# lmb-freiburg/demon

Measured on NVIDIA H100. Metric: image_pairs_per_sec_256x192, higher is better.
Workload: dtype tf32x3

## Files before the change

### demon_b200/_lib.py

```python
import ctypes
import os

_HERE = os.path.dirname(os.path.abspath(__file__))
_DEFAULT = os.path.join(_HERE, "lib", "libdemon_b200.so")

c_void_p, c_int, c_int64, c_float, c_double, c_char_p = (
    ctypes.c_void_p, ctypes.c_int, ctypes.c_int64, ctypes.c_float, ctypes.c_double, ctypes.c_char_p)

_P = c_void_p
PROTOTYPES = {
    "demon_warp2d_f32": [_P, _P, _P, c_int, c_int, c_int, c_int, c_int, c_int, c_float, _P],
    "demon_warp2d_f64": [_P, _P, _P, c_int, c_int, c_int, c_int, c_int, c_int, c_double, _P],
    "demon_depth_to_flow_f32": [_P, _P, _P, _P, _P, c_int, c_int, c_int, c_int, c_int, c_int, _P],
    "demon_depth_to_flow_f64": [_P, _P, _P, _P, _P, c_int, c_int, c_int, c_int, c_int, c_int, _P],
    "demon_flow_to_depth_f32": [_P, _P, _P, _P, _P, c_int, c_int, c_int, c_int, c_int, c_int, _P],
    "demon_flow_to_depth_f64": [_P, _P, _P, _P, _P, c_int, c_int, c_int, c_int, c_int, c_int, _P],
    "demon_leaky_relu_f32": [_P, _P, c_int64, c_float, _P],
    "demon_leaky_relu_f64": [_P, _P, c_int64, c_double, _P],
    "demon_median3x3_downsample_f32": [_P, _P, c_int64, c_int, c_int, _P],
    "demon_median3x3_downsample_f64": [_P, _P, c_int64, c_int, c_int, _P],
    "demon_scale_invariant_gradient_f32": [_P, _P, c_int64, c_int, c_int, _P, _P, c_int, c_float, _P],
    "demon_scale_invariant_gradient_f64": [_P, _P, c_int64, c_int, c_int, _P, _P, c_int, c_double, _P],
    "demon_scale_invariant_gradient_grad_f32": [_P, _P, _P, c_int64, c_int, c_int, _P, _P, c_int, c_float, _P],
    "demon_scale_invariant_gradient_grad_f64": [_P, _P, _P, c_int64, c_int, c_int, _P, _P, c_int, c_double, _P],
# ... 82 lines not shown
    "demon_net_batch": [_P],
    "demon_net_workspace_bytes": [_P],
    "demon_net_pipeline_launches": [_P, c_int],
    "demon_net_snapshot_launches": [_P, c_int],
    "demon_net_layer_uses_tensor_cores": [_P, c_char_p],
    "demon_net_profile_begin": [_P],
    "demon_net_profile_end": [_P],
    "demon_net_num_layers": [_P],
    "demon_net_layer_name": [_P, c_int],
    "demon_net_layer_profile": [_P, c_int, _P, _P, _P, _P],
    "demon_debug_tc_timeouts": [],
    "demon_check_errors": [],
    "demon_debug_describe_layers": [_P, _P, c_int],
    "demon_debug_trace_layers": [_P, _P, _P],
    "demon_debug_describe_conv": [c_int] * 13 + [_P, c_int],
    "demon_debug_last_conv_ms": [],
    "demon_debug_tc_timing": [c_int, _P, c_int],
    "demon_conv_slice_nhwc": [_P, c_int, _P] + [c_int] * 11 + [_P, _P, c_int, c_int, _P],
    "demon_conv_slice_nhwc_same": [_P, c_int, _P] + [c_int] * 10 + [_P, _P, c_int, c_int, _P],
    "demon_conv2d_nhwc": [_P, _P] + [c_int] * 9 + [_P, _P, c_int, c_int, _P],
    "demon_deconv4x4s2_nhwc": [_P, _P] + [c_int] * 5 + [_P, _P, c_int, c_int, _P],
    "demon_last_error": [],
    "demon_version": [],
    "demon_launch_count": [],
}
_RESTYPES = {
    "demon_net_destroy": None,
    "demon_net_variable_name": c_char_p,
    "demon_net_layer_name": c_char_p,
    "demon_net_workspace_bytes": c_int64,
# ... 47 lines not shown
```

### demon_b200/csrc/conv_tc.cuh

```cuda
#pragma once
#include "conv.cuh"

namespace demon {

struct HaloPlan;

struct TcLayer {
  HaloPlan* plan = nullptr;
  size_t splitk_bytes = 0;
  bool per_tap = false;
};

constexpr int kTcNoPlan = 1;

int tc_prepare(TcLayer& t, const ConvProblem* probs, const float* const* w_hosts, int nclass, int precision);
int conv_tc_launch(const TcLayer& t, const ConvProblem* probs, cudaStream_t stream);
int tc_describe(const ConvProblem* probs, int nclass, int precision, char* buf, int buflen);
void tc_layer_free(TcLayer& t);
int tc_read_error_flag(bool clear);
void tc_halo_enable_timing(bool on);
int tc_halo_read_timing(long long* host, int nblocks);

}
```

### demon_b200/csrc/conv_tc_halo.cu

```cuda
#include <cuda.h>

#include <algorithm>
#include <cstring>
#include <memory>
#include <mutex>
#include <vector>

#include "conv_tc.cuh"
#include "conv_tc_ptx.cuh"
#include "wgmma_tf32.cuh"

namespace demon {

namespace {

constexpr int kRing = 4;
constexpr int kThreads = 384;
constexpr int kConsumerWarps = 8;
constexpr int kMaxAStages = 4;
constexpr int kTileH = 16, kTileW = 8;
constexpr int kMaxPlanes = 4;
constexpr int kPlanSms = 132;
constexpr int kSmemBudget = 224 * 1024;
constexpr int kMaxDynSmem = 226 * 1024;
// ... 48 lines not shown
__device__ __forceinline__ void wait_t(uint32_t bar, uint32_t parity, int* err, long long& acc) {
  if (mbar_try(bar, parity)) return;
  const long long t0 = clock64();
  for (;;) {
    if (mbar_try(bar, parity)) break;
    if (clock64() - t0 > kTimeoutCycles || *reinterpret_cast<volatile int*>(err) != 0) {
      atomicExch(err, 1);
      break;
    }
  }
  acc += clock64() - t0;
}

__device__ __forceinline__ int fast_div(int x, int d, uint32_t mul) { return mul ? (int)__umulhi((uint32_t)x, mul) : x; }

template <bool PER_TAP>
__device__ __forceinline__ void halo_decode_tile(const HaloParams& p, int tile, int& nt, int& n, int& y0, int& x0) {
  int m = fast_div(tile, p.n_tiles, p.mul_n_tiles);
  nt = tile - m * p.n_tiles;
  const int m1 = fast_div(m, p.tiles_x, p.mul_tiles_x);
  const int xb = m - m1 * p.tiles_x;
  n = fast_div(m1, p.tiles_y, p.mul_tiles_y);
  const int yb = m1 - n * p.tiles_y;
  if (PER_TAP) { n *= p.tb; y0 = yb * p.th; x0 = xb * p.tw; }
  else { y0 = yb * kTileH; x0 = xb * kTileW; }
}

template <int N, int MODE>
__device__ __forceinline__ void issue_block(float* acc, const uint32_t* hi, const uint32_t* lo, uint32_t wb) {
  const uint64_t w_hi = wgmma_desc_sw128(wb);
  const uint64_t w_lo = wgmma_desc_sw128(wb + N * 128u);
#pragma unroll
  for (int j = 0; j < 4; ++j) {
    if (MODE == 2) {
      Wgmma<N>::mma(acc, hi[4 * j], hi[4 * j + 1], hi[4 * j + 2], hi[4 * j + 3], w_lo + (uint64_t)(2 * j));
      Wgmma<N>::mma(acc, lo[4 * j], lo[4 * j + 1], lo[4 * j + 2], lo[4 * j + 3], w_hi + (uint64_t)(2 * j));
    }
    Wgmma<N>::mma(acc, hi[4 * j], hi[4 * j + 1], hi[4 * j + 2], hi[4 * j + 3], w_hi + (uint64_t)(2 * j));
  }
}

template <bool PER_TAP, bool CIN8, int MODE, int N, int NCLS>
__global__ void __launch_bounds__(kThreads, 1) conv_tc_halo_kernel(const __grid_constant__ HaloMaps maps, const HaloParams p) {
  extern __shared__ __align__(1024) unsigned char smem_raw[];
  unsigned char* smem = reinterpret_cast<unsigned char*>((reinterpret_cast<uintptr_t>(smem_raw) + 1023) & ~(uintptr_t)1023);
  __shared__ __align__(8) uint64_t bars[2 * kMaxAStages + 2 * kRing + 1];

  const int warp = threadIdx.x >> 5;
  const int lane = threadIdx.x & 31;
  const uint32_t afull0 = smem_u32(&bars[0]), aempty0 = smem_u32(&bars[kMaxAStages]);
  const uint32_t wfull0 = smem_u32(&bars[2 * kMaxAStages]), wempty0 = smem_u32(&bars[2 * kMaxAStages + kRing]);
  const uint32_t wres_bar = smem_u32(&bars[2 * kMaxAStages + 2 * kRing]);
  const int a_stage_bytes = p.a_region_bytes;
  unsigned char* w_ring = smem + (size_t)p.sa * a_stage_bytes;

  if (warp == 0 && lane == 0) {
    for (int i = 0; i < p.nplanes; ++i) asm volatile("prefetch.tensormap [%0];" ::"l"(&maps.m[i]) : "memory");
    for (int s = 0; s < kMaxAStages; ++s) {
// ... 19 lines not shown
    if (p.w_resident) {
      const uint32_t total = (uint32_t)(p.k_chunks * p.w_chunk_bytes);
      mbar_expect_tx(wres_bar, total);
      for (int kc = 0; kc < p.k_chunks; ++kc)
        bulk_load(smem_u32(w_ring + (size_t)kc * p.w_chunk_bytes), p.w + (size_t)kc * p.w_chunk_bytes, (uint32_t)p.w_chunk_bytes, wres_bar);
    }
    uint32_t a_bytes = 0;
    for (int i = 0; i < p.nplanes; ++i) a_bytes += (uint32_t)p.planes[i].bytes;
    int sa = 0, slot = 0;
    uint32_t pa = 0, use = 0;
    pdl_wait();
    for (int item = blockIdx.x; item < p.total_items; item += gridDim.x) {
      const int tile = fast_div(item, p.ksplit, p.mul_ksplit);
      const int kc0 = (item - tile * p.ksplit) * p.kc_split;
      int nt, n, y0, x0;
      halo_decode_tile<PER_TAP>(p, tile, nt, n, y0, x0);
      const unsigned char* wsrc = p.w + ((size_t)nt * p.k_chunks + kc0) * p.w_chunk_bytes;
      for (int kc = kc0; kc < kc0 + p.kc_split; ++kc, wsrc += p.w_chunk_bytes) {
        if (!PER_TAP) {
          wait_t(aempty0 + 8 * sa, pa ^ 1, p.err, w_aempty);
          const uint32_t abase = smem_u32(smem + (size_t)sa * a_stage_bytes);
          mbar_expect_tx(afull0 + 8 * sa, a_bytes);
          for (int i = 0; i < p.nplanes; ++i) {
            const HaloPlane& pl = p.planes[i];
            tma_load_5d(abase + pl.smem_off, &maps.m[i], afull0 + 8 * sa, pl.c_off + kc * 32, x0 + pl.qx_min, pl.ry, y0 + pl.qy_min, n);
          }
          if (++sa == p.sa) { sa = 0; pa ^= 1; }
        }
        for (int t = 0; t < p.nsteps; ++t) {
          if (PER_TAP) {
            wait_t(aempty0 + 8 * sa, pa ^ 1, p.err, w_aempty);
// ... 8 lines not shown
            mbar_expect_tx(wfull0 + 8 * slot, bytes);
            bulk_load(smem_u32(w_ring + (size_t)slot * p.w_stage_bytes), wsrc + p.st_woff[t], bytes, wfull0 + 8 * slot);
            if (++slot == kRing) { slot = 0; use ^= 1; }
          }
        }
      }
    }
    if (timed) { p.timing[blockIdx.x * 16 + 0] = w_aempty; p.timing[blockIdx.x * 16 + 1] = w_wempty; p.timing[blockIdx.x * 16 + 8] = clock64() - t_begin; }
    return;
  }

  asm volatile("setmaxnreg.inc.sync.aligned.u32 232;");
  const int wg = (warp >> 2) - 1;
  const int wq = warp & 3;
  const int g = lane >> 2, tq = lane & 3;
  const int m0 = 64 * wg + 16 * wq + g;
  int pos_y[2], pos_x[2], pos_n[2];
#pragma unroll
  for (int h = 0; h < 2; ++h) {
    const int m = m0 + 8 * h;
    pos_x[h] = PER_TAP ? (m % p.tw) : (m & 7);
    pos_y[h] = PER_TAP ? ((m / p.tw) % p.th) : (m >> 3);
    pos_n[h] = PER_TAP ? (m / (p.tw * p.th)) : 0;
  }
  const float slope = p.leaky ? 0.1f : 1.0f;
  const uint32_t w_ring_u = smem_u32(w_ring);
  long long w_afull = 0, w_wfull = 0;
  const long long t_begin = clock64();
  int sa = 0, slot = 0, l_res = 0;
  uint32_t pa = 0, use = 0;
  if (p.w_resident) wait_t(wres_bar, 0u, p.err, w_wfull);
  pdl_wait();
  float acc[NCLS][N / 2];
  for (int item = blockIdx.x; item < p.total_items; item += gridDim.x) {
    const int tile = fast_div(item, p.ksplit, p.mul_ksplit);
    const int z = item - tile * p.ksplit;
    int nt, n, y0, x0;
    halo_decode_tile<PER_TAP>(p, tile, nt, n, y0, x0);
#pragma unroll
    for (int k = 0; k < NCLS; ++k)
#pragma unroll
      for (int i = 0; i < N / 2; ++i) acc[k][i] = 0.f;
    l_res = 0;
    for (int kc = 0; kc < p.kc_split; ++kc) {
      uint32_t abase = 0;
      if (!PER_TAP) {
        wait_t(afull0 + 8 * sa, pa, p.err, w_afull);
        abase = smem_u32(smem + (size_t)sa * a_stage_bytes);
      }
      for (int t = 0; t < p.nsteps; ++t) {
        if (PER_TAP) {
          wait_t(afull0 + 8 * sa, pa, p.err, w_afull);
          abase = smem_u32(smem + (size_t)sa * a_stage_bytes);
        }
        float v[2][8];
#pragma unroll
        for (int h = 0; h < 2; ++h) {
          if (CIN8) {
            const int rt = 4 * t + tq;
            const int pi = (rt < p.ntaps_real) ? p.g_plane[rt] : -1;
            float4 a = make_float4(0.f, 0.f, 0.f, 0.f), b = a;
            if (pi >= 0) {
              const HaloPlane& pl = p.planes[pi];
              const uint32_t px = abase + (uint32_t)(pl.smem_off + p.g_aoff[rt] + (pos_y[h] * pl.cols + pos_x[h]) * 32);
              a = lds128(px); b = lds128(px + 16);
            }
            v[h][0] = a.x; v[h][1] = a.y; v[h][2] = a.z; v[h][3] = a.w; v[h][4] = b.x; v[h][5] = b.y; v[h][6] = b.z; v[h][7] = b.w;
          } else {
            uint32_t row;
            if (PER_TAP) {
              row = abase + (uint32_t)((m0 + 8 * h) * 128);
            } else {
              const HaloPlane& pl = p.planes[p.st_plane[t]];
              row = abase + (uint32_t)(pl.smem_off + p.st_aoff[t] + (pos_y[h] * pl.cols + pos_x[h]) * 128);
            }
            const uint32_t phase = (row >> 7) & 7u;
            const float4 a = lds128(row + (((uint32_t)(2 * tq) ^ phase) << 4));
            const float4 b = lds128(row + (((uint32_t)(2 * tq + 1) ^ phase) << 4));
            v[h][0] = a.x; v[h][1] = a.y; v[h][2] = a.z; v[h][3] = a.w; v[h][4] = b.x; v[h][5] = b.y; v[h][6] = b.z; v[h][7] = b.w;
          }
        }
        uint32_t hi[16], lo[16];
#pragma unroll
        for (int j = 0; j < 4; ++j) {
          const float f[4] = {v[0][2 * j], v[1][2 * j], v[0][2 * j + 1], v[1][2 * j + 1]};
#pragma unroll
          for (int e = 0; e < 4; ++e) {
            const uint32_t u = __float_as_uint(f[e]);
            hi[4 * j + e] = (MODE == 2) ? (u & 0xFFFFE000u) : u;
            lo[4 * j + e] = __float_as_uint(f[e] - __uint_as_float(u & 0xFFFFE000u));
          }
        }
        uint32_t wb;
        if (p.w_resident) {
          wb = w_ring_u + (uint32_t)(l_res++) * (uint32_t)p.w_stage_bytes;
        } else {
          wait_t(wfull0 + 8 * slot, use, p.err, w_wfull);
          wb = w_ring_u + (uint32_t)slot * (uint32_t)p.w_stage_bytes;
        }
#pragma unroll
        for (int k = 0; k < NCLS; ++k)
#pragma unroll
          for (int i = 0; i < N / 2; ++i) reg_fence(acc[k][i]);
        wgmma_fence();
        if (NCLS == 1) {
          issue_block<N, MODE>(acc[0], hi, lo, wb);
        } else {
          const uint32_t cm = (uint32_t)p.st_cmask[t];
#pragma unroll
          for (int k = 0; k < NCLS; ++k)
            if (cm & (1u << k)) {
              issue_block<N, MODE>(acc[k], hi, lo, wb);
              wb += (uint32_t)p.cls_bytes;
            }
        }
        wgmma_commit();
        wgmma_wait0();
#pragma unroll
        for (int k = 0; k < NCLS; ++k)
#pragma unroll
          for (int i = 0; i < N / 2; ++i) reg_fence(acc[k][i]);
        __syncwarp();
        if (lane == 0) {
          if (!p.w_resident) mbar_arrive(wempty0 + 8 * slot);
          if (PER_TAP) mbar_arrive(aempty0 + 8 * sa);
        }
        if (!p.w_resident && ++slot == kRing) { slot = 0; use ^= 1; }
        if (PER_TAP && ++sa == p.sa) { sa = 0; pa ^= 1; }
      }
      if (!PER_TAP) {
        __syncwarp();
        if (lane == 0) mbar_arrive(aempty0 + 8 * sa);
        if (++sa == p.sa) { sa = 0; pa ^= 1; }
      }
    }
    float* tile_out = p.out + (size_t)z * p.part_stride + ((size_t)(n * p.Hfull + y0 * p.osy) * p.Wfull + x0 * p.osx) * p.out_pitch;
    const int cbase = nt * N;
#pragma unroll
    for (int k = 0; k < NCLS; ++k) {
      if (k >= p.nclass) break;
      float* cls_out = tile_out + (size_t)(p.cls_ooy[k] * p.Wfull + p.cls_oox[k]) * p.out_pitch;
#pragma unroll
      for (int h = 0; h < 2; ++h) {
        if (y0 + pos_y[h] >= p.Ho || x0 + pos_x[h] >= p.Wo || n + pos_n[h] >= p.B) continue;
        float* orow = cls_out + ((size_t)(pos_n[h] * p.Hfull + pos_y[h] * p.osy) * p.Wfull + pos_x[h] * p.osx) * p.out_pitch;
#pragma unroll
        for (int i = 0; i < N / 8; ++i) {
          const int col = cbase + 8 * i + 2 * tq;
          if (col >= p.Cout) continue;
          const float2 b = p.bias ? __ldg(reinterpret_cast<const float2*>(p.bias + col)) : make_float2(0.f, 0.f);
          float2 o;
          o.x = acc[k][4 * i + 2 * h] + b.x;
          o.y = acc[k][4 * i + 2 * h + 1] + b.y;
          o.x = fmaxf(slope * o.x, o.x); o.y = fmaxf(slope * o.y, o.y);
          *reinterpret_cast<float2*>(orow + col) = o;
        }
      }
    }
  }
  if (timed && threadIdx.x == 128) { p.timing[blockIdx.x * 16 + 6] = w_afull; p.timing[blockIdx.x * 16 + 3] = w_wfull; p.timing[blockIdx.x * 16 + 9] = clock64() - t_begin; }
}

__global__ void __launch_bounds__(256) halo_splitk_reduce_kernel(const float* __restrict__ part, long long part_stride, int ksplit,
                                                                 float* __restrict__ out, int out_pitch, int cpitch, int Cout, long long npix,
                                                                 const float* __restrict__ bias, int leaky) {
  pdl_launch_dependents();
  pdl_wait();
  const int c4n = cpitch >> 2;
// ... 10 lines not shown
    }
    acc.x = fmaxf(slope * acc.x, acc.x); acc.y = fmaxf(slope * acc.y, acc.y);
    acc.z = fmaxf(slope * acc.z, acc.z); acc.w = fmaxf(slope * acc.w, acc.w);
    *reinterpret_cast<float4*>(out + (size_t)pix * out_pitch + c) = acc;
  }
}

int floor_div_h(int a, int b) { return (a >= 0) ? a / b : -((-a + b - 1) / b); }

}

struct HaloPlan {
  HaloParams prm;
  HaloMaps maps;
  int smem_bytes;
  int st_tap[kMaxTaps][4];
};

static int pow2_ceil_h(int v) { int r = 1; while (r < v) r <<= 1; return r; }
static int popcount4(int m) { return (m & 1) + ((m >> 1) & 1) + ((m >> 2) & 1) + ((m >> 3) & 1); }

struct ShiftStep { int ry, rx, qy, qx, cmask, tap[4]; };

static bool halo_build(const ConvProblem* probs, int nclass, int nsplit, HaloPlan& plan, bool force_per_tap) {
  const ConvProblem& p = probs[0];
  HaloParams& prm = plan.prm;
  const int budget = kSmemBudget;
  struct Cand { int max_cls, n_cap; };
  std::vector<Cand> cands;
  for (int mc = nclass; mc >= 1; mc = (mc > 2 ? 2 : mc - 1)) cands.push_back({mc, 256});
  cands.push_back({1, 64});
  cands.push_back({1, 32});
  bool found = false;
  for (const Cand& cand : cands) {
    const int max_cls = cand.max_cls;
    memset(&prm, 0, sizeof(prm));
    memset(plan.st_tap, -1, sizeof(plan.st_tap));
    prm.nclass = nclass;
    prm.nsplit = nsplit;
    prm.cin8 = (p.Cin == 8) ? 1 : 0;
    const int px_bytes = prm.cin8 ? 32 : 128;
// ... 44 lines not shown
        for (size_t k = 0; k < pinfo.size(); ++k)
          if (pinfo[k].ry == steps[t].ry && pinfo[k].rx == steps[t].rx) pi = (int)k;
        if (pi < 0) { pinfo.push_back({steps[t].ry, steps[t].rx, steps[t].qy, steps[t].qy, steps[t].qx, steps[t].qx}); pi = (int)pinfo.size() - 1; }
        PInfo& pl = pinfo[pi];
        pl.qy_min = std::min(pl.qy_min, steps[t].qy); pl.qy_max = std::max(pl.qy_max, steps[t].qy);
        pl.qx_min = std::min(pl.qx_min, steps[t].qx); pl.qx_max = std::max(pl.qx_max, steps[t].qx);
        step_plane[t] = pi;
      }
      if ((int)pinfo.size() > kMaxPlanes) return false;
      prm.nplanes = (int)pinfo.size();
      int off = 0;
      for (int i = 0; i < prm.nplanes; ++i) {
        HaloPlane& pl = prm.planes[i];
        pl.c_off = pinfo[i].rx * p.in_pitch; pl.ry = pinfo[i].ry;
        pl.qx_min = pinfo[i].qx_min; pl.qy_min = pinfo[i].qy_min;
        pl.cols = kTileW + pinfo[i].qx_max - pinfo[i].qx_min;
        pl.rows = kTileH + pinfo[i].qy_max - pinfo[i].qy_min;
        if (pl.cols > 256 || pl.rows > 256) return false;
        pl.bytes = pl.rows * pl.cols * px_bytes;
        pl.smem_off = off;
        off += (pl.bytes + 1023) / 1024 * 1024;
      }
      prm.a_region_bytes = off;
      for (int t = 0; t < nreal; ++t) {
        const HaloPlane& pl = prm.planes[step_plane[t]];
        prm.st_plane[t] = step_plane[t];
        prm.st_aoff[t] = ((steps[t].qy - pl.qy_min) * pl.cols + (steps[t].qx - pl.qx_min)) * px_bytes;
      }
      prm.tiles_x = ceil_div(p.Wo, kTileW); prm.tiles_y = ceil_div(p.Ho, kTileH); prm.tiles_b = p.B;
      m_tiles = prm.tiles_x * prm.tiles_y * p.B;
    }
    for (int t = 0; t < nreal; ++t) {
      prm.st_cmask[t] = steps[t].cmask;
      for (int c = 0; c < 4; ++c) plan.st_tap[t][c] = steps[t].tap[c];
    }
    prm.nsteps = nreal;
    if (prm.cin8) {
      prm.ntaps_real = nreal;
      for (int t = 0; t < nreal; ++t) { prm.g_plane[t] = prm.st_plane[t]; prm.g_aoff[t] = prm.st_aoff[t]; }
      prm.nsteps = (nreal + 3) / 4;
      for (int t = 0; t < prm.nsteps; ++t) { prm.st_plane[t] = 0; prm.st_aoff[t] = 0; prm.st_cmask[t] = 1; }
    }
    const int cout16 = (p.Cout + 15) / 16 * 16;
    int n_tile = std::min(pow2_ceil_h(std::max(cout16, 16)), std::min(nclass > 1 ? 64 : 128, cand.n_cap));
// ... 20 lines not shown
      prm.w_resident = 1;
      prm.w_region_bytes = w_total;
    }
    const int rest = budget - prm.w_region_bytes;
    if (rest < 2 * prm.a_region_bytes) continue;
    prm.sa = std::min(kMaxAStages, rest / prm.a_region_bytes);
    plan.smem_bytes = prm.sa * prm.a_region_bytes + prm.w_region_bytes + 1024;
    found = true;
    break;
  }
  if (!found || prm.sa < 2) return false;
  prm.B = p.B;
  const int m_tiles = prm.tiles_x * prm.tiles_y * prm.tiles_b;
  prm.total_tiles = m_tiles * prm.n_tiles;
  prm.ksplit = 1;
  if (!prm.cin8 && !prm.w_resident && prm.k_chunks >= 4) {
    const long out_bytes = (long)p.B * p.Hfull * p.Wfull * ((p.Cout + 3) / 4 * 4) * 4;
    auto cost = [&](int ks) {
      const long items = (long)prm.total_tiles * ks;
      return ((items + kPlanSms - 1) / kPlanSms) * ((long)(prm.k_chunks / ks) * prm.nsteps * 600 + 3000) + (ks > 1 ? 12000 + ks * out_bytes * 2 / 4000 : 0);
    };
    long best = cost(1);
    for (int ks = 2; ks <= 8; ++ks) {
      if (prm.k_chunks % ks != 0 || prm.k_chunks / ks < 2) continue;
      const long c = cost(ks);
      if (c * 10 < best * 9 && c < cost(prm.ksplit)) prm.ksplit = ks;
    }
  }
  prm.kc_split = prm.k_chunks / prm.ksplit;
  prm.total_items = prm.total_tiles * prm.ksplit;
  prm.part_stride = 0;
// ... 9 lines not shown
}

static bool tc_shape_supported(const ConvProblem& p) {
  const bool cin8 = p.Cin == 8 && p.in_pitch == 8;
  if (!cin8 && (p.Cin < 32 || (p.Cin % 32) != 0)) return false;
  if (p.Cout < 16 || (p.Cout % 4) != 0) return false;
  if ((p.in_pitch % 4) != 0 || (p.out_pitch % 4) != 0) return false;
  if ((reinterpret_cast<uintptr_t>(p.in) & 15) != 0 || (reinterpret_cast<uintptr_t>(p.out) & 15) != 0) return false;
  if (p.sy < 1 || p.sx < 1 || (p.Hi % p.sy) != 0 || (p.Wi % p.sx) != 0) return false;
  if (p.ntaps < 1 || p.ntaps > kMaxTaps) return false;
  if (p.scale != nullptr) return false;
  if (p.Ho != p.Hi / p.sy || p.Wo != p.Wi / p.sx) return false;
  return true;
}

static bool tc_plan(const ConvProblem* probs, int nclass, int nsplit, HaloPlan& plan) {
  if (nclass < 1 || nclass > 4) return false;
  for (int c = 0; c < nclass; ++c) {
    if (!tc_shape_supported(probs[c])) return false;
    if (probs[c].in != probs[0].in || probs[c].Cout != probs[0].Cout || probs[c].sy != probs[0].sy || probs[c].sx != probs[0].sx) return false;
  }
  return halo_build(probs, nclass, nsplit, plan, false) || halo_build(probs, nclass, nsplit, plan, true);
}

static int nsplit_of(int precision) { return (precision == DEMON_PREC_TF32) ? 1 : 3; }

static bool encode_maps(const ConvProblem& p, HaloPlan& plan) {
  const HaloParams& prm = plan.prm;
  typedef CUresult (*EncodeTiledFn)(CUtensorMap*, CUtensorMapDataType, cuuint32_t, void*, const cuuint64_t*, const cuuint64_t*,
                                    const cuuint32_t*, const cuuint32_t*, CUtensorMapInterleave, CUtensorMapSwizzle,
                                    CUtensorMapL2promotion, CUtensorMapFloatOOBfill);
  void* fp = nullptr;
  cudaDriverEntryPointQueryResult qres;
  if (cudaGetDriverEntryPoint("cuTensorMapEncodeTiled", &fp, cudaEnableDefault, &qres) != cudaSuccess || qres != cudaDriverEntryPointSuccess)
    return false;
  EncodeTiledFn enc = reinterpret_cast<EncodeTiledFn>(fp);
  const cuuint64_t cp = (cuuint64_t)p.in_pitch;
// ... 2 lines not shown
  cuuint64_t gstr[4] = {(cuuint64_t)p.sx * cp * 4, (cuuint64_t)p.Wi * cp * 4, (cuuint64_t)p.sy * p.Wi * cp * 4,
                        (cuuint64_t)p.Hi * p.Wi * cp * 4};
  cuuint32_t estr[5] = {1, 1, 1, 1, 1};
  for (int i = 0; i < prm.nplanes; ++i) {
    cuuint32_t box[5] = {(cuuint32_t)(prm.cin8 ? 8 : 32), (cuuint32_t)prm.planes[i].cols, 1, (cuuint32_t)prm.planes[i].rows,
                         (cuuint32_t)(prm.per_tap ? prm.tb : 1)};
    CUresult r = enc(&plan.maps.m[i], CU_TENSOR_MAP_DATA_TYPE_FLOAT32, 5, const_cast<float*>(p.in), gdim, gstr, box, estr,
                     CU_TENSOR_MAP_INTERLEAVE_NONE, prm.cin8 ? CU_TENSOR_MAP_SWIZZLE_NONE : CU_TENSOR_MAP_SWIZZLE_128B,
                     CU_TENSOR_MAP_L2_PROMOTION_L2_256B, CU_TENSOR_MAP_FLOAT_OOB_FILL_NONE);
    if (r != CUDA_SUCCESS) return false;
  }
  for (int i = prm.nplanes; i < kMaxPlanes; ++i) plan.maps.m[i] = plan.maps.m[0];
  return true;
}

int tc_describe(const ConvProblem* probs, int nclass, int precision, char* buf, int buflen) {
  HaloPlan plan;
  if (!tc_plan(probs, nclass, nsplit_of(precision), plan)) return 0;
  const HaloParams& q = plan.prm;
  int n = snprintf(buf, buflen,
                   "halo %s mode %d n_tile %d x%d steps %d x %d chunks sa %d a_stage %d w_slot %d smem %d tiles %d ksplit %d wres %d tb %d th %d tw %d |",
                   q.per_tap ? "per-tap" : (q.cin8 ? "cin8" : "halo"), q.mode, q.n_tile, q.n_tiles, q.nsteps, q.k_chunks, q.sa,
                   q.a_region_bytes, q.w_stage_bytes, plan.smem_bytes, q.total_tiles, q.ksplit, q.w_resident, q.per_tap ? q.tb : 1,
                   q.per_tap ? q.th : kTileH, q.per_tap ? q.tw : kTileW);
  for (int t = 0; t < q.nsteps && n < buflen - 32; ++t)
    n += snprintf(buf + n, buflen - n, " [c%x w%d+%d]", q.st_cmask[t], q.st_woff[t], q.st_wbytes[t]);
  return n;
}

static float tf32_round_h(float x) {
  uint32_t u;
  memcpy(&u, &x, 4);
  if ((u & 0x7F800000u) == 0x7F800000u) return x;
  u += 0x00000FFFu + ((u >> 13) & 1u);
  u &= 0xFFFFE000u;
  float r;
  memcpy(&r, &u, 4);
  return r;
}
// ... 94 lines not shown
  return v;
}

static long long* g_timing_dev = nullptr;
void tc_halo_enable_timing(bool on) {
  if (on && !g_timing_dev) { cudaMalloc(&g_timing_dev, 256 * 16 * sizeof(long long)); }
  if (g_timing_dev) cudaMemset(g_timing_dev, 0, 256 * 16 * sizeof(long long));
  if (!on && g_timing_dev) { cudaFree(g_timing_dev); g_timing_dev = nullptr; }
}
int tc_halo_read_timing(long long* host, int nblocks) {
  if (!g_timing_dev) return -1;
  cudaMemcpy(host, g_timing_dev, (size_t)nblocks * 16 * sizeof(long long), cudaMemcpyDeviceToHost);
  return 0;
}

template <bool PER_TAP, bool CIN8, int MODE, int N, int NCLS>
static int launch_variant(const HaloPlan* plan, const HaloParams& prm, int grid, cudaStream_t stream) {
  TcDeviceState& ds = tc_device_state();
  static int attr_device = -1;
  if (attr_device != ds.device) {
    DEMON_CHECK_CUDA(cudaFuncSetAttribute(conv_tc_halo_kernel<PER_TAP, CIN8, MODE, N, NCLS>, cudaFuncAttributeMaxDynamicSharedMemorySize, kMaxDynSmem));
    attr_device = ds.device;
  }
  cudaError_t le = launch_pdl(conv_tc_halo_kernel<PER_TAP, CIN8, MODE, N, NCLS>, dim3(grid), dim3(kThreads), (size_t)plan->smem_bytes, stream, plan->maps, prm);
  if (le != cudaSuccess) return fail(DEMON_E_CUDA, "conv_tc_halo launch: %s", cudaGetErrorString(le));
  DEMON_LAUNCH_CHECK();
  return DEMON_OK;
}

template <bool PER_TAP, bool CIN8, int MODE, int NCLS>
static int launch_n(const HaloPlan* plan, const HaloParams& prm, int grid, cudaStream_t stream) {
  switch (prm.n_tile) {
    case 16: return launch_variant<PER_TAP, CIN8, MODE, 16, NCLS>(plan, prm, grid, stream);
    case 32: return launch_variant<PER_TAP, CIN8, MODE, 32, NCLS>(plan, prm, grid, stream);
    case 64: return launch_variant<PER_TAP, CIN8, MODE, 64, NCLS>(plan, prm, grid, stream);
    default: break;
  }
  if (NCLS == 1 && prm.n_tile == 128) return launch_variant<PER_TAP, CIN8, MODE, (NCLS == 1 ? 128 : 64), NCLS>(plan, prm, grid, stream);
  return fail(DEMON_E_STATE, "conv_tc_halo: no kernel for N tile %d with %d classes", prm.n_tile, prm.nclass);
}

template <bool PER_TAP, bool CIN8, int NCLS>
static int launch_mode(const HaloPlan* plan, const HaloParams& prm, int grid, cudaStream_t stream) {
  return prm.mode == 0 ? launch_n<PER_TAP, CIN8, 0, NCLS>(plan, prm, grid, stream) : launch_n<PER_TAP, CIN8, 2, NCLS>(plan, prm, grid, stream);
}

// ... 38 lines not shown
```

### demon_b200/csrc/conv_tc_ptx.cuh

```cuda
#pragma once
#include <cuda.h>
#include <cstdint>

namespace demon {
namespace {

constexpr long long kTimeoutCycles = 4000000000ll;

__device__ __forceinline__ uint32_t smem_u32(const void* p) { return (uint32_t)__cvta_generic_to_shared(p); }

__device__ __forceinline__ void mbar_init(uint32_t bar, uint32_t count) {
  asm volatile("mbarrier.init.shared::cta.b64 [%0], %1;" ::"r"(bar), "r"(count));
}
__device__ __forceinline__ void mbar_arrive(uint32_t bar) {
  asm volatile("{\n.reg .b64 st;\nmbarrier.arrive.shared::cta.b64 st, [%0];\n}" ::"r"(bar) : "memory");
}
__device__ __forceinline__ void mbar_expect_tx(uint32_t bar, uint32_t bytes) {
  asm volatile("{\n.reg .b64 st;\nmbarrier.arrive.expect_tx.shared::cta.b64 st, [%0], %1;\n}" ::"r"(bar), "r"(bytes) : "memory");
}
__device__ __forceinline__ bool mbar_try(uint32_t bar, uint32_t parity) {
  uint32_t done;
  asm volatile(
      "{\n.reg .pred p;\n"
      "mbarrier.try_wait.parity.shared::cta.b64 p, [%1], %2;\n"
// ... 7 lines not shown
__device__ __forceinline__ void tma_load_5d(uint32_t dst, const CUtensorMap* map, uint32_t bar, int c0, int c1, int c2, int c3, int c4) {
  asm volatile(
      "cp.async.bulk.tensor.5d.shared::cluster.global.mbarrier::complete_tx::bytes [%0], [%1, {%3, %4, %5, %6, %7}], [%2];"
      ::"r"(dst), "l"(map), "r"(bar), "r"(c0), "r"(c1), "r"(c2), "r"(c3), "r"(c4)
      : "memory");
}
__device__ __forceinline__ void bulk_load(uint32_t dst, const void* src, uint32_t bytes, uint32_t bar) {
  asm volatile("cp.async.bulk.shared::cluster.global.mbarrier::complete_tx::bytes [%0], [%1], %2, [%3];" ::"r"(dst), "l"(src),
               "r"(bytes), "r"(bar)
               : "memory");
}
__device__ __forceinline__ void wgmma_fence() { asm volatile("wgmma.fence.sync.aligned;" ::: "memory"); }
__device__ __forceinline__ void wgmma_commit() { asm volatile("wgmma.commit_group.sync.aligned;" ::: "memory"); }
__device__ __forceinline__ void wgmma_wait0() { asm volatile("wgmma.wait_group.sync.aligned 0;" ::: "memory"); }
__device__ __forceinline__ void reg_fence(float& x) { asm volatile("" : "+f"(x)::"memory"); }

__device__ __forceinline__ uint64_t wgmma_desc_sw128(uint32_t smem_addr) {
  uint64_t d = 0;
  d |= (uint64_t)((smem_addr & 0x3FFFF) >> 4);
  d |= (uint64_t)1 << 16;
  d |= (uint64_t)(1024 >> 4) << 32;
  d |= (uint64_t)1 << 62;
  return d;
}

__device__ __forceinline__ bool elect_one_sync() {
  uint32_t pred;
  asm volatile("{\n.reg .b32 rx;\n.reg .pred px;\nelect.sync rx|px, 0xffffffff;\nselp.b32 %0, 1, 0, px;\n}" : "=r"(pred));
  return pred != 0;
}
// ... 9 lines not shown
```

### demon_b200/csrc/net.cu

```cuda
#include <algorithm>
#include <cstdlib>
#include <cstring>
#include <map>
#include <memory>
#include <string>
#include <type_traits>
#include <vector>

#include "conv.cuh"
#include "conv_tc.cuh"
#include "geometry.cuh"
#include "images.cuh"

namespace demon {

namespace {

struct Buf {
  float* p = nullptr;
  int H = 0, W = 0, C = 0;
  size_t offset = 0;
  size_t numel(int B) const { return (size_t)B * H * W * C; }
};

// ... 1646 lines not shown
  n->trace_in.assign(L, nullptr);
  n->trace_out.assign(L, nullptr);
  if (in) std::copy(in, in + L, n->trace_in.begin());
  if (out) std::copy(out, out + L, n->trace_out.begin());
  n->tracing = in || out;
  return DEMON_OK;
}

int demon_debug_describe_conv(int B, int H, int W, int Cin, int in_pitch, int Cout, int out_pitch, int kh, int kw, int sy, int sx, int deconv,
                              int precision, char* buf, int buflen) {
  DEMON_REQUIRE(buf && buflen > 0, "describe: null");
  StandaloneLayer s(nullptr, nullptr, H, W, Cin, in_pitch, Cout, out_pitch, kh, kw, sy, sx, deconv != 0, false);
  return describe_layer(s.layer, B, precision, buf, buflen);
}

static double g_last_conv_ms = -1.0;
double demon_debug_last_conv_ms(void) { return g_last_conv_ms; }

static int standalone_conv(const float* in, int in_pitch, float* out, int out_pitch, int B, int H, int W, int Cin, int Cout, int kh, int kw,
                           int sy, int sx, const float* kernel_host, const float* bias_host, int leaky, int precision, bool deconv, void* stream,
                           bool tf_same = false) {
  DEMON_REQUIRE(in && out && kernel_host && bias_host, "conv: null pointer");
  DEMON_REQUIRE(Cin % 4 == 0, "conv test entry: Cin must be a multiple of 4");
  DEMON_REQUIRE(B >= 1 && H >= 1 && W >= 1 && Cout >= 1 && in_pitch >= Cin && out_pitch >= Cout, "conv test entry: shape or pitch");
  if (deconv) DEMON_REQUIRE(kh == 4 && kw == 4 && sy == 2 && sx == 2, "deconv: only k4 s2");
  else DEMON_REQUIRE(kh >= 1 && kw >= 1 && kh * kw <= kMaxTaps && (kh & 1) && (kw & 1), "conv: kernel %dx%d", kh, kw);
  DEMON_REQUIRE(sy >= 1 && sx >= 1, "conv: stride");
  std::vector<void*> allocs;
  StandaloneLayer s(in, out, H, W, Cin, in_pitch, Cout, out_pitch, kh, kw, sy, sx, deconv, leaky != 0);
  Layer& l = s.layer;
// ... 57 lines not shown
```

### include/demon_b200.h

```cpp
#ifndef DEMON_B200_H
#define DEMON_B200_H

#include <stdint.h>

#ifdef __cplusplus
extern "C" {
#endif

#define DEMON_OK            0
#define DEMON_E_INVALID    -1
#define DEMON_E_CUDA       -2
#define DEMON_E_STATE      -3
#define DEMON_E_NOTFOUND   -4

#define DEMON_BORDER_CLAMP  1
#define DEMON_BORDER_VALUE  2
#define DEMON_ROT_MATRIX     0
#define DEMON_ROT_QUATERNION 1
#define DEMON_ROT_ANGLEAXIS3 2

const char* demon_last_error(void);
const char* demon_version(void);
int64_t demon_launch_count(void);

// ... 299 lines not shown
int demon_net_layer_profile(const demon_net* net, int i, double* ms, int64_t* calls, int* launches_per_call,
                            int* uses_tc);

int demon_debug_tc_timeouts(void);
int demon_check_errors(void);
int demon_debug_tc_timing(int enable, int64_t* host_out, int nblocks);

int demon_debug_describe_layers(const demon_net* net, char* buf, int buflen);
int demon_debug_describe_plan(int variant, int batch, int refine_h, int refine_w, int precision, char* buf, int buflen);

int demon_debug_trace_layers(demon_net* net, float* const* in, float* const* out);

int demon_debug_describe_conv(int B, int H, int W, int Cin, int in_pitch, int Cout, int out_pitch, int kh, int kw, int sy, int sx,
                              int deconv, int precision, char* buf, int buflen);

double demon_debug_last_conv_ms(void);

int demon_conv_slice_nhwc(const float* in, int in_pitch, float* out, int out_pitch, int B, int H, int W, int Cin, int Cout,
                          int kh, int kw, int sy, int sx, int deconv, const float* kernel_host, const float* bias_host,
                          int leaky, int precision, void* stream);

int demon_conv_slice_nhwc_same(const float* in, int in_pitch, float* out, int out_pitch, int B, int H, int W, int Cin, int Cout,
                               int kh, int kw, int sy, int sx, const float* kernel_host, const float* bias_host,
                               int leaky, int precision, void* stream);

int demon_conv2d_nhwc(const float* in, float* out, int B, int H, int W, int Cin, int Cout,
                      int kh, int kw, int sy, int sx, const float* kernel_host, const float* bias_host,
                      int leaky, int precision, void* stream);
int demon_deconv4x4s2_nhwc(const float* in, float* out, int B, int H, int W, int Cin, int Cout,
                           const float* kernel_host, const float* bias_host, int leaky, int precision,
// ... 7 lines not shown
```

Baseline: 2861.

## Add two-row-block halo conv tiles to reuse weight descriptors across wider M

Adds an MB template parameter to the halo tensor-core conv kernel so each consumer warpgroup computes two 64-row M blocks (tile width doubled to 16) per weight fetch. This reuses the same weight stage across two wgmma sequences, which amortises weight traffic and synchronisation per MMA. The planner enables it only for halo mode with N tile up to 32 and when the tile count stays balanced across SMs. It doubles accumulator and fragment registers and enlarges the halo smem planes, and a debug API toggles the behaviour.

```diff
diff --git a/demon_b200/_lib.py b/demon_b200/_lib.py
--- a/demon_b200/_lib.py
+++ b/demon_b200/_lib.py
@@ -120,6 +120,7 @@
     "demon_debug_describe_layers": [_P, _P, c_int],
     "demon_debug_trace_layers": [_P, _P, _P],
     "demon_debug_describe_conv": [c_int] * 13 + [_P, c_int],
+    "demon_debug_tc_max_row_blocks": [c_int],
     "demon_debug_last_conv_ms": [],
     "demon_debug_tc_timing": [c_int, _P, c_int],
     "demon_conv_slice_nhwc": [_P, c_int, _P] + [c_int] * 11 + [_P, _P, c_int, c_int, _P],
diff --git a/demon_b200/csrc/conv_tc.cuh b/demon_b200/csrc/conv_tc.cuh
--- a/demon_b200/csrc/conv_tc.cuh
+++ b/demon_b200/csrc/conv_tc.cuh
@@ -16,6 +16,7 @@
 int tc_prepare(TcLayer& t, const ConvProblem* probs, const float* const* w_hosts, int nclass, int precision);
 int conv_tc_launch(const TcLayer& t, const ConvProblem* probs, cudaStream_t stream);
 int tc_describe(const ConvProblem* probs, int nclass, int precision, char* buf, int buflen);
+int tc_set_max_row_blocks(int mb);
 void tc_layer_free(TcLayer& t);
 int tc_read_error_flag(bool clear);
 void tc_halo_enable_timing(bool on);
diff --git a/demon_b200/csrc/conv_tc_halo.cu b/demon_b200/csrc/conv_tc_halo.cu
--- a/demon_b200/csrc/conv_tc_halo.cu
+++ b/demon_b200/csrc/conv_tc_halo.cu
@@ -86,7 +86,7 @@
 
 __device__ __forceinline__ int fast_div(int x, int d, uint32_t mul) { return mul ? (int)__umulhi((uint32_t)x, mul) : x; }
 
-template <bool PER_TAP>
+template <bool PER_TAP, int MB>
 __device__ __forceinline__ void halo_decode_tile(const HaloParams& p, int tile, int& nt, int& n, int& y0, int& x0) {
   int m = fast_div(tile, p.n_tiles, p.mul_n_tiles);
   nt = tile - m * p.n_tiles;
@@ -95,25 +95,32 @@
   n = fast_div(m1, p.tiles_y, p.mul_tiles_y);
   const int yb = m1 - n * p.tiles_y;
   if (PER_TAP) { n *= p.tb; y0 = yb * p.th; x0 = xb * p.tw; }
-  else { y0 = yb * kTileH; x0 = xb * kTileW; }
-}
-
-template <int N, int MODE>
-__device__ __forceinline__ void issue_block(float* acc, const uint32_t* hi, const uint32_t* lo, uint32_t wb) {
+  else { y0 = yb * kTileH; x0 = xb * (kTileW * MB); }
+}
+
+template <int N, int MODE, int MB>
+__device__ __forceinline__ void issue_block(float* const* acc, const uint32_t (*hi)[16], const uint32_t (*lo)[16], uint32_t wb) {
   const uint64_t w_hi = wgmma_desc_sw128(wb);
   const uint64_t w_lo = wgmma_desc_sw128(wb + N * 128u);
 #pragma unroll
   for (int j = 0; j < 4; ++j) {
     if (MODE == 2) {
-      Wgmma<N>::mma(acc, hi[4 * j], hi[4 * j + 1], hi[4 * j + 2], hi[4 * j + 3], w_lo + (uint64_t)(2 * j));
-      Wgmma<N>::mma(acc, lo[4 * j], lo[4 * j + 1], lo[4 * j + 2], lo[4 * j + 3], w_hi + (uint64_t)(2 * j));
-    }
-    Wgmma<N>::mma(acc, hi[4 * j], hi[4 * j + 1], hi[4 * j + 2], hi[4 * j + 3], w_hi + (uint64_t)(2 * j));
-  }
-}
-
-template <bool PER_TAP, bool CIN8, int MODE, int N, int NCLS>
+#pragma unroll
+      for (int b = 0; b < MB; ++b)
+        Wgmma<N>::mma(acc[b], hi[b][4 * j], hi[b][4 * j + 1], hi[b][4 * j + 2], hi[b][4 * j + 3], w_lo + (uint64_t)(2 * j));
+#pragma unroll
+      for (int b = 0; b < MB; ++b)
+        Wgmma<N>::mma(acc[b], lo[b][4 * j], lo[b][4 * j + 1], lo[b][4 * j + 2], lo[b][4 * j + 3], w_hi + (uint64_t)(2 * j));
+    }
+#pragma unroll
+    for (int b = 0; b < MB; ++b)
+      Wgmma<N>::mma(acc[b], hi[b][4 * j], hi[b][4 * j + 1], hi[b][4 * j + 2], hi[b][4 * j + 3], w_hi + (uint64_t)(2 * j));
+  }
+}
+
+template <bool PER_TAP, bool CIN8, int MODE, int N, int NCLS, int MB>
 __global__ void __launch_bounds__(kThreads, 1) conv_tc_halo_kernel(const __grid_constant__ HaloMaps maps, const HaloParams p) {
+  static_assert(MB == 1 || (!PER_TAP && !CIN8 && N <= 32), "row blocks: halo mode, N <= 32");
   extern __shared__ __align__(1024) unsigned char smem_raw[];
   unsigned char* smem = reinterpret_cast<unsigned char*>((reinterpret_cast<uintptr_t>(smem_raw) + 1023) & ~(uintptr_t)1023);
   __shared__ __align__(8) uint64_t bars[2 * kMaxAStages + 2 * kRing + 1];
@@ -163,7 +170,7 @@
       const int tile = fast_div(item, p.ksplit, p.mul_ksplit);
       const int kc0 = (item - tile * p.ksplit) * p.kc_split;
       int nt, n, y0, x0;
-      halo_decode_tile<PER_TAP>(p, tile, nt, n, y0, x0);
+      halo_decode_tile<PER_TAP, MB>(p, tile, nt, n, y0, x0);
       const unsigned char* wsrc = p.w + ((size_t)nt * p.k_chunks + kc0) * p.w_chunk_bytes;
       for (int kc = kc0; kc < kc0 + p.kc_split; ++kc, wsrc += p.w_chunk_bytes) {
         if (!PER_TAP) {
@@ -202,15 +209,17 @@
   const int wg = (warp >> 2) - 1;
   const int wq = warp & 3;
   const int g = lane >> 2, tq = lane & 3;
-  const int m0 = 64 * wg + 16 * wq + g;
-  int pos_y[2], pos_x[2], pos_n[2];
-#pragma unroll
-  for (int h = 0; h < 2; ++h) {
-    const int m = m0 + 8 * h;
-    pos_x[h] = PER_TAP ? (m % p.tw) : (m & 7);
-    pos_y[h] = PER_TAP ? ((m / p.tw) % p.th) : (m >> 3);
-    pos_n[h] = PER_TAP ? (m / (p.tw * p.th)) : 0;
-  }
+  const int m0 = 64 * MB * wg + 16 * wq + g;
+  int pos_y[MB][2], pos_x[MB][2], pos_n[MB][2];
+#pragma unroll
+  for (int b = 0; b < MB; ++b)
+#pragma unroll
+    for (int h = 0; h < 2; ++h) {
+      const int m = m0 + 64 * b + 8 * h;
+      pos_x[b][h] = PER_TAP ? (m % p.tw) : (m & (kTileW * MB - 1));
+      pos_y[b][h] = PER_TAP ? ((m / p.tw) % p.th) : (m >> (MB + 2));
+      pos_n[b][h] = PER_TAP ? (m / (p.tw * p.th)) : 0;
+    }
   const float slope = p.leaky ? 0.1f : 1.0f;
   const uint32_t w_ring_u = smem_u32(w_ring);
   long long w_afull = 0, w_wfull = 0;
@@ -219,16 +228,18 @@
   uint32_t pa = 0, use = 0;
   if (p.w_resident) wait_t(wres_bar, 0u, p.err, w_wfull);
   pdl_wait();
-  float acc[NCLS][N / 2];
+  float acc[MB][NCLS][N / 2];
   for (int item = blockIdx.x; item < p.total_items; item += gridDim.x) {
     const int tile = fast_div(item, p.ksplit, p.mul_ksplit);
     const int z = item - tile * p.ksplit;
     int nt, n, y0, x0;
-    halo_decode_tile<PER_TAP>(p, tile, nt, n, y0, x0);
-#pragma unroll
-    for (int k = 0; k < NCLS; ++k)
-#pragma unroll
-      for (int i = 0; i < N / 2; ++i) acc[k][i] = 0.f;
+    halo_decode_tile<PER_TAP, MB>(p, tile, nt, n, y0, x0);
+#pragma unroll
+    for (int b = 0; b < MB; ++b)
+#pragma unroll
+      for (int k = 0; k < NCLS; ++k)
+#pragma unroll
+        for (int i = 0; i < N / 2; ++i) acc[b][k][i] = 0.f;
     l_res = 0;
     for (int kc = 0; kc < p.kc_split; ++kc) {
       uint32_t abase = 0;
@@ -241,7 +252,9 @@
           wait_t(afull0 + 8 * sa, pa, p.err, w_afull);
           abase = smem_u32(smem + (size_t)sa * a_stage_bytes);
         }
-        float v[2][8];
+        float v[MB][2][8];
+#pragma unroll
+        for (int rb = 0; rb < MB; ++rb)
 #pragma unroll
         for (int h = 0; h < 2; ++h) {
           if (CIN8) {
@@ -250,33 +263,35 @@
             float4 a = make_float4(0.f, 0.f, 0.f, 0.f), b = a;
             if (pi >= 0) {
               const HaloPlane& pl = p.planes[pi];
-              const uint32_t px = abase + (uint32_t)(pl.smem_off + p.g_aoff[rt] + (pos_y[h] * pl.cols + pos_x[h]) * 32);
+              const uint32_t px = abase + (uint32_t)(pl.smem_off + p.g_aoff[rt] + (pos_y[rb][h] * pl.cols + pos_x[rb][h]) * 32);
               a = lds128(px); b = lds128(px + 16);
             }
-            v[h][0] = a.x; v[h][1] = a.y; v[h][2] = a.z; v[h][3] = a.w; v[h][4] = b.x; v[h][5] = b.y; v[h][6] = b.z; v[h][7] = b.w;
+            v[rb][h][0] = a.x; v[rb][h][1] = a.y; v[rb][h][2] = a.z; v[rb][h][3] = a.w; v[rb][h][4] = b.x; v[rb][h][5] = b.y; v[rb][h][6] = b.z; v[rb][h][7] = b.w;
           } else {
             uint32_t row;
             if (PER_TAP) {
               row = abase + (uint32_t)((m0 + 8 * h) * 128);
             } else {
               const HaloPlane& pl = p.planes[p.st_plane[t]];
-              row = abase + (uint32_t)(pl.smem_off + p.st_aoff[t] + (pos_y[h] * pl.cols + pos_x[h]) * 128);
+              row = abase + (uint32_t)(pl.smem_off + p.st_aoff[t] + (pos_y[rb][h] * pl.cols + pos_x[rb][h]) * 128);
             }
             const uint32_t phase = (row >> 7) & 7u;
             const float4 a = lds128(row + (((uint32_t)(2 * tq) ^ phase) << 4));
             const float4 b = lds128(row + (((uint32_t)(2 * tq + 1) ^ phase) << 4));
-            v[h][0] = a.x; v[h][1] = a.y; v[h][2] = a.z; v[h][3] = a.w; v[h][4] = b.x; v[h][5] = b.y; v[h][6] = b.z; v[h][7] = b.w;
+            v[rb][h][0] = a.x; v[rb][h][1] = a.y; v[rb][h][2] = a.z; v[rb][h][3] = a.w; v[rb][h][4] = b.x; v[rb][h][5] = b.y; v[rb][h][6] = b.z; v[rb][h][7] = b.w;
           }
         }
-        uint32_t hi[16], lo[16];
+        uint32_t hi[MB][16], lo[MB][16];
+#pragma unroll
+        for (int rb = 0; rb < MB; ++rb)
 #pragma unroll
         for (int j = 0; j < 4; ++j) {
-          const float f[4] = {v[0][2 * j], v[1][2 * j], v[0][2 * j + 1], v[1][2 * j + 1]};
+          const float f[4] = {v[rb][0][2 * j], v[rb][1][2 * j], v[rb][0][2 * j + 1], v[rb][1][2 * j + 1]};
 #pragma unroll
           for (int e = 0; e < 4; ++e) {
             const uint32_t u = __float_as_uint(f[e]);
-            hi[4 * j + e] = (MODE == 2) ? (u & 0xFFFFE000u) : u;
-            lo[4 * j + e] = __float_as_uint(f[e] - __uint_as_float(u & 0xFFFFE000u));
+            hi[rb][4 * j + e] = (MODE == 2) ? (u & 0xFFFFE000u) : u;
+            lo[rb][4 * j + e] = __float_as_uint(f[e] - __uint_as_float(u & 0xFFFFE000u));
           }
         }
         uint32_t wb;
@@ -287,27 +302,43 @@
           wb = w_ring_u + (uint32_t)slot * (uint32_t)p.w_stage_bytes;
         }
 #pragma unroll
+        for (int rb = 0; rb < MB; ++rb)
+#pragma unroll
         for (int k = 0; k < NCLS; ++k)
 #pragma unroll
-          for (int i = 0; i < N / 2; ++i) reg_fence(acc[k][i]);
+          for (int i = 0; i < N / 2; ++i) reg_fence(acc[rb][k][i]);
+        if (MB == 2) {
+#pragma unroll
+          for (int rb = 0; rb < MB; ++rb)
+#pragma unroll
+            for (int i = 0; i < 16; ++i) { reg_fence_u(hi[rb][i]); reg_fence_u(lo[rb][i]); }
+        }
         wgmma_fence();
         if (NCLS == 1) {
-          issue_block<N, MODE>(acc[0], hi, lo, wb);
+          float* blocks[MB];
+#pragma unroll
+          for (int rb = 0; rb < MB; ++rb) blocks[rb] = acc[rb][0];
+          issue_block<N, MODE, MB>(blocks, hi, lo, wb);
         } else {
           const uint32_t cm = (uint32_t)p.st_cmask[t];
 #pragma unroll
           for (int k = 0; k < NCLS; ++k)
             if (cm & (1u << k)) {
-              issue_block<N, MODE>(acc[k], hi, lo, wb);
+              float* blocks[MB];
+#pragma unroll
+              for (int rb = 0; rb < MB; ++rb) blocks[rb] = acc[rb][k];
+              issue_block<N, MODE, MB>(blocks, hi, lo, wb);
               wb += (uint32_t)p.cls_bytes;
             }
         }
         wgmma_commit();
         wgmma_wait0();
 #pragma unroll
+        for (int rb = 0; rb < MB; ++rb)
+#pragma unroll
         for (int k = 0; k < NCLS; ++k)
 #pragma unroll
-          for (int i = 0; i < N / 2; ++i) reg_fence(acc[k][i]);
+          for (int i = 0; i < N / 2; ++i) reg_fence(acc[rb][k][i]);
         __syncwarp();
         if (lane == 0) {
           if (!p.w_resident) mbar_arrive(wempty0 + 8 * slot);
@@ -329,17 +360,19 @@
       if (k >= p.nclass) break;
       float* cls_out = tile_out + (size_t)(p.cls_ooy[k] * p.Wfull + p.cls_oox[k]) * p.out_pitch;
 #pragma unroll
+      for (int rb = 0; rb < MB; ++rb)
+#pragma unroll
       for (int h = 0; h < 2; ++h) {
-        if (y0 + pos_y[h] >= p.Ho || x0 + pos_x[h] >= p.Wo || n + pos_n[h] >= p.B) continue;
-        float* orow = cls_out + ((size_t)(pos_n[h] * p.Hfull + pos_y[h] * p.osy) * p.Wfull + pos_x[h] * p.osx) * p.out_pitch;
+        if (y0 + pos_y[rb][h] >= p.Ho || x0 + pos_x[rb][h] >= p.Wo || n + pos_n[rb][h] >= p.B) continue;
+        float* orow = cls_out + ((size_t)(pos_n[rb][h] * p.Hfull + pos_y[rb][h] * p.osy) * p.Wfull + pos_x[rb][h] * p.osx) * p.out_pitch;
 #pragma unroll
         for (int i = 0; i < N / 8; ++i) {
           const int col = cbase + 8 * i + 2 * tq;
           if (col >= p.Cout) continue;
           const float2 b = p.bias ? __ldg(reinterpret_cast<const float2*>(p.bias + col)) : make_float2(0.f, 0.f);
           float2 o;
-          o.x = acc[k][4 * i + 2 * h] + b.x;
-          o.y = acc[k][4 * i + 2 * h + 1] + b.y;
+          o.x = acc[rb][k][4 * i + 2 * h] + b.x;
+          o.y = acc[rb][k][4 * i + 2 * h + 1] + b.y;
           o.x = fmaxf(slope * o.x, o.x); o.y = fmaxf(slope * o.y, o.y);
           *reinterpret_cast<float2*>(orow + col) = o;
         }
@@ -380,6 +413,7 @@
   HaloParams prm;
   HaloMaps maps;
   int smem_bytes;
+  int mb;
   int st_tap[kMaxTaps][4];
 };
 
@@ -388,9 +422,10 @@
 
 struct ShiftStep { int ry, rx, qy, qx, cmask, tap[4]; };
 
-static bool halo_build(const ConvProblem* probs, int nclass, int nsplit, HaloPlan& plan, bool force_per_tap) {
+static bool halo_build(const ConvProblem* probs, int nclass, int nsplit, HaloPlan& plan, bool force_per_tap, int mb) {
   const ConvProblem& p = probs[0];
   HaloParams& prm = plan.prm;
+  plan.mb = mb;
   const int budget = kSmemBudget;
   struct Cand { int max_cls, n_cap; };
   std::vector<Cand> cands;
@@ -465,7 +500,7 @@
         HaloPlane& pl = prm.planes[i];
         pl.c_off = pinfo[i].rx * p.in_pitch; pl.ry = pinfo[i].ry;
         pl.qx_min = pinfo[i].qx_min; pl.qy_min = pinfo[i].qy_min;
-        pl.cols = kTileW + pinfo[i].qx_max - pinfo[i].qx_min;
+        pl.cols = kTileW * mb + pinfo[i].qx_max - pinfo[i].qx_min;
         pl.rows = kTileH + pinfo[i].qy_max - pinfo[i].qy_min;
         if (pl.cols > 256 || pl.rows > 256) return false;
         pl.bytes = pl.rows * pl.cols * px_bytes;
@@ -478,7 +513,8 @@
         prm.st_plane[t] = step_plane[t];
         prm.st_aoff[t] = ((steps[t].qy - pl.qy_min) * pl.cols + (steps[t].qx - pl.qx_min)) * px_bytes;
       }
-      prm.tiles_x = ceil_div(p.Wo, kTileW); prm.tiles_y = ceil_div(p.Ho, kTileH); prm.tiles_b = p.B;
+      prm.tb = 1; prm.th = kTileH; prm.tw = kTileW * mb;
+      prm.tiles_x = ceil_div(p.Wo, prm.tw); prm.tiles_y = ceil_div(p.Ho, kTileH); prm.tiles_b = p.B;
       m_tiles = prm.tiles_x * prm.tiles_y * p.B;
     }
     for (int t = 0; t < nreal; ++t) {
@@ -529,7 +565,11 @@
   const int m_tiles = prm.tiles_x * prm.tiles_y * prm.tiles_b;
   prm.total_tiles = m_tiles * prm.n_tiles;
   prm.ksplit = 1;
-  if (!prm.cin8 && !prm.w_resident && prm.k_chunks >= 4) {
+  if (mb == 2) {
+    if (prm.per_tap || prm.cin8 || (nclass == 1 ? prm.n_tile > 32 : prm.n_tile != 32)) return false;
+    if (7 * ceil_div(prm.total_tiles, kPlanSms) >= 4 * ceil_div(2 * prm.total_tiles, kPlanSms)) return false;
+  }
+  if (!prm.cin8 && !prm.w_resident && prm.k_chunks >= 4 && mb == 1) {
     const long out_bytes = (long)p.B * p.Hfull * p.Wfull * ((p.Cout + 3) / 4 * 4) * 4;
     auto cost = [&](int ks) {
       const long items = (long)prm.total_tiles * ks;
@@ -569,13 +609,20 @@
   return true;
 }
 
+static int g_max_row_blocks = 2;
+
 static bool tc_plan(const ConvProblem* probs, int nclass, int nsplit, HaloPlan& plan) {
   if (nclass < 1 || nclass > 4) return false;
   for (int c = 0; c < nclass; ++c) {
     if (!tc_shape_supported(probs[c])) return false;
     if (probs[c].in != probs[0].in || probs[c].Cout != probs[0].Cout || probs[c].sy != probs[0].sy || probs[c].sx != probs[0].sx) return false;
   }
-  return halo_build(probs, nclass, nsplit, plan, false) || halo_build(probs, nclass, nsplit, plan, true);
+  if (!halo_build(probs, nclass, nsplit, plan, false, 1)) return halo_build(probs, nclass, nsplit, plan, true, 1);
+  HaloPlan two;
+  if (g_max_row_blocks >= 2 && !plan.prm.per_tap && probs[0].Wo % (2 * kTileW) == 0 && halo_build(probs, nclass, nsplit, two, false, 2) &&
+      two.prm.n_tile == plan.prm.n_tile && two.prm.w_resident == plan.prm.w_resident)
+    plan = two;
+  return true;
 }
 
 static int nsplit_of(int precision) { return (precision == DEMON_PREC_TF32) ? 1 : 3; }
@@ -608,6 +655,12 @@
   return true;
 }
 
+int tc_set_max_row_blocks(int mb) {
+  const int prev = g_max_row_blocks;
+  g_max_row_blocks = (mb >= 2) ? 2 : 1;
+  return prev;
+}
+
 int tc_describe(const ConvProblem* probs, int nclass, int precision, char* buf, int buflen) {
   HaloPlan plan;
   if (!tc_plan(probs, nclass, nsplit_of(precision), plan)) return 0;
@@ -616,7 +669,7 @@
                    "halo %s mode %d n_tile %d x%d steps %d x %d chunks sa %d a_stage %d w_slot %d smem %d tiles %d ksplit %d wres %d tb %d th %d tw %d |",
                    q.per_tap ? "per-tap" : (q.cin8 ? "cin8" : "halo"), q.mode, q.n_tile, q.n_tiles, q.nsteps, q.k_chunks, q.sa,
                    q.a_region_bytes, q.w_stage_bytes, plan.smem_bytes, q.total_tiles, q.ksplit, q.w_resident, q.per_tap ? q.tb : 1,
-                   q.per_tap ? q.th : kTileH, q.per_tap ? q.tw : kTileW);
+                   q.per_tap ? q.th : kTileH, q.per_tap ? q.tw : kTileW * plan.mb);
   for (int t = 0; t < q.nsteps && n < buflen - 32; ++t)
     n += snprintf(buf + n, buflen - n, " [c%x w%d+%d]", q.st_cmask[t], q.st_woff[t], q.st_wbytes[t]);
   return n;
@@ -741,15 +794,15 @@
   return 0;
 }
 
-template <bool PER_TAP, bool CIN8, int MODE, int N, int NCLS>
+template <bool PER_TAP, bool CIN8, int MODE, int N, int NCLS, int MB = 1>
 static int launch_variant(const HaloPlan* plan, const HaloParams& prm, int grid, cudaStream_t stream) {
   TcDeviceState& ds = tc_device_state();
   static int attr_device = -1;
   if (attr_device != ds.device) {
-    DEMON_CHECK_CUDA(cudaFuncSetAttribute(conv_tc_halo_kernel<PER_TAP, CIN8, MODE, N, NCLS>, cudaFuncAttributeMaxDynamicSharedMemorySize, kMaxDynSmem));
+    DEMON_CHECK_CUDA(cudaFuncSetAttribute(conv_tc_halo_kernel<PER_TAP, CIN8, MODE, N, NCLS, MB>, cudaFuncAttributeMaxDynamicSharedMemorySize, kMaxDynSmem));
     attr_device = ds.device;
   }
-  cudaError_t le = launch_pdl(conv_tc_halo_kernel<PER_TAP, CIN8, MODE, N, NCLS>, dim3(grid), dim3(kThreads), (size_t)plan->smem_bytes, stream, plan->maps, prm);
+  cudaError_t le = launch_pdl(conv_tc_halo_kernel<PER_TAP, CIN8, MODE, N, NCLS, MB>, dim3(grid), dim3(kThreads), (size_t)plan->smem_bytes, stream, plan->maps, prm);
   if (le != cudaSuccess) return fail(DEMON_E_CUDA, "conv_tc_halo launch: %s", cudaGetErrorString(le));
   DEMON_LAUNCH_CHECK();
   return DEMON_OK;
@@ -757,6 +810,16 @@
 
 template <bool PER_TAP, bool CIN8, int MODE, int NCLS>
 static int launch_n(const HaloPlan* plan, const HaloParams& prm, int grid, cudaStream_t stream) {
+  if (plan->mb == 2) {
+    if constexpr (!PER_TAP && !CIN8 && NCLS == 4) {
+      if (prm.n_tile == 32) return launch_variant<PER_TAP, CIN8, MODE, 32, NCLS, 2>(plan, prm, grid, stream);
+    }
+    if constexpr (!PER_TAP && !CIN8 && NCLS == 1) {
+      if (prm.n_tile == 16) return launch_variant<PER_TAP, CIN8, MODE, 16, NCLS, 2>(plan, prm, grid, stream);
+      if (prm.n_tile == 32) return launch_variant<PER_TAP, CIN8, MODE, 32, NCLS, 2>(plan, prm, grid, stream);
+    }
+    return fail(DEMON_E_STATE, "conv_tc_halo: no kernel for two row blocks at N tile %d with %d classes", prm.n_tile, prm.nclass);
+  }
   switch (prm.n_tile) {
     case 16: return launch_variant<PER_TAP, CIN8, MODE, 16, NCLS>(plan, prm, grid, stream);
     case 32: return launch_variant<PER_TAP, CIN8, MODE, 32, NCLS>(plan, prm, grid, stream);
diff --git a/demon_b200/csrc/conv_tc_ptx.cuh b/demon_b200/csrc/conv_tc_ptx.cuh
--- a/demon_b200/csrc/conv_tc_ptx.cuh
+++ b/demon_b200/csrc/conv_tc_ptx.cuh
@@ -45,6 +45,7 @@
 __device__ __forceinline__ void wgmma_commit() { asm volatile("wgmma.commit_group.sync.aligned;" ::: "memory"); }
 __device__ __forceinline__ void wgmma_wait0() { asm volatile("wgmma.wait_group.sync.aligned 0;" ::: "memory"); }
 __device__ __forceinline__ void reg_fence(float& x) { asm volatile("" : "+f"(x)::"memory"); }
+__device__ __forceinline__ void reg_fence_u(uint32_t& x) { asm volatile("" : "+r"(x)::"memory"); }
 
 __device__ __forceinline__ uint64_t wgmma_desc_sw128(uint32_t smem_addr) {
   uint64_t d = 0;
diff --git a/demon_b200/csrc/net.cu b/demon_b200/csrc/net.cu
--- a/demon_b200/csrc/net.cu
+++ b/demon_b200/csrc/net.cu
@@ -1684,6 +1684,11 @@
   return describe_layer(s.layer, B, precision, buf, buflen);
 }
 
+int demon_debug_tc_max_row_blocks(int mb) {
+  DEMON_REQUIRE(mb == 1 || mb == 2, "row blocks: 1 or 2");
+  return tc_set_max_row_blocks(mb);
+}
+
 static double g_last_conv_ms = -1.0;
 double demon_debug_last_conv_ms(void) { return g_last_conv_ms; }
 
diff --git a/include/demon_b200.h b/include/demon_b200.h
--- a/include/demon_b200.h
+++ b/include/demon_b200.h
@@ -337,6 +337,8 @@
 int demon_debug_describe_conv(int B, int H, int W, int Cin, int in_pitch, int Cout, int out_pitch, int kh, int kw, int sy, int sx,
                               int deconv, int precision, char* buf, int buflen);
 
+int demon_debug_tc_max_row_blocks(int mb);
+
 double demon_debug_last_conv_ms(void);
 
 int demon_conv_slice_nhwc(const float* in, int in_pitch, float* out, int out_pitch, int B, int H, int W, int Cin, int Cout,
```

Result: faster. 2946 (median of 6 runs) (+3.0%).
